# LGMOak/HighPerformanceComputing-LatticeBoltzmannMethod

Measured on NVIDIA B200. Metric: MLUPS (fp64 D2Q9), higher is better.
Workload: dtype f64

## Files before the change

highperformancecomputing-latticeboltzmannmethod_b200/csrc/lbm_tb.cu:

```cuda
#include <cstdlib>

#include "lbm_device.cuh"
#include "lbm_launch.cuh"
#include "lbm_tb.cuh"

namespace lbm {

namespace {

#ifndef TB_SKEW_THREADS
#define TB_SKEW_THREADS 512
#endif

template <int T, int B, bool FORCED, bool SKEW, bool FUSED>
__device__ __forceinline__ void tb_kernel_body(const TbArgs& a, int p2p) {
    extern __shared__ double ring[];
    pdl_wait();
    pdl_release();
    const bool edge_block = p2p && blockIdx.y < 2;
    if (edge_block) p2p_block_begin(a.px);
    tb_thread<T, B, FORCED, SKEW, FUSED>(a, ring, threadIdx.x, blockIdx.x, blockIdx.y);
    if (edge_block) p2p_block_end(a.px, gridDim.x * 2);
}

template <int T, int B, bool FORCED, bool SKEW = true, bool FUSED = false>
__global__ void __launch_bounds__(B, (T == 3 ? 384 : ((SKEW && T == 2) || T == 1 ? TB_SKEW_THREADS : 768)) / B)
    k_tb(const __grid_constant__ TbArgs a, int p2p) {
    tb_kernel_body<T, B, FORCED, SKEW, FUSED>(a, p2p);
}

__global__ void __launch_bounds__(256) k_macros_finish(ObserveArgs o, const double* __restrict__ m_rho,
                                                       const double* __restrict__ m_ux, const double* __restrict__ m_uy,
                                                       double* __restrict__ rho, double* __restrict__ ux,
                                                       double* __restrict__ uy) {
    __shared__ double t[3][32][33];
    const Layout& L = o.L;
    const int x0 = blockIdx.y * 32, y0 = blockIdx.x * 32;
    for (int k = threadIdx.y; k < 32; k += blockDim.y) {
        const int x = x0 + k, y = y0 + threadIdx.x;
        if (x < L.lnx && y < L.ny) {
            const long long g = (long long)x * L.ny + y;
            double r = m_rho[g], u = m_ux[g], v = m_uy[g];
            const bool on_in = o.bc.inlet && x == 0, on_out = o.bc.outlet && x == L.lnx - 1;
            if ((on_in || on_out) && !o.mask[L.at(x + 1, y)]) {
                double f[Q], rb = 0.0, uo = 0.0;
                current_from_next(o.cur, L, o.mask, o.bc, x, y, f, rb, uo);
                if (on_in) { r = rb; u = o.bc.u_in; v = 0.0; }
                if (on_out) { r = 1.0; u = uo; v = 0.0; }
            }
            t[0][k][threadIdx.x] = r;
            t[1][k][threadIdx.x] = u;
            t[2][k][threadIdx.x] = v;
        }
    }
    __syncthreads();
    for (int k = threadIdx.y; k < 32; k += blockDim.y) {
        const int x = x0 + threadIdx.x, y = y0 + k;
        if (x < L.lnx && y < L.ny) {
            const long long g = (long long)y * L.lnx + x;
            rho[g] = t[0][threadIdx.x][k];
            ux[g] = t[1][threadIdx.x][k];
            uy[g] = t[2][threadIdx.x][k];
        }
    }
}

inline int cdiv(long long a, long long b) { return (int)((a + b - 1) / b); }

int env_int(const char* name, int dflt) {
    const char* v = std::getenv(name);
    return v ? std::atoi(v) : dflt;
}

template <int T, int B, bool FORCED, bool SKEW = true, bool FUSED = false>
cudaError_t launch_one(TbArgs a, bool p2p, cudaStream_t s) {
    using S = TbShape<T, B>;
    auto kern = k_tb<T, B, FORCED, SKEW, FUSED>;
    const size_t smem = (size_t)S::RING_DOUBLES * sizeof(double) + (FUSED ? 16 : 0);
    static int slots = 0;
    if (!slots) {
        if (smem > 48 * 1024) {
            cudaError_t e = cudaFuncSetAttribute(kern, cudaFuncAttributeMaxDynamicSharedMemorySize, (int)smem);
            if (e != cudaSuccess) return e;
        }
        int per_sm = 0, dev = 0, sms = 0;
        cudaGetDevice(&dev);
        cudaDeviceGetAttribute(&sms, cudaDevAttrMultiProcessorCount, dev);
        cudaError_t e = cudaOccupancyMaxActiveBlocksPerMultiprocessor(&per_sm, kern, B, smem);
        if (e != cudaSuccess) return e;
        slots = (per_sm > 0 ? per_sm : 1) * (sms > 0 ? sms : 1);
    }
    const int lnx = a.L.lnx;
    const int strips = cdiv(a.L.ny, S::H);
    a.edge_cols = 0;
    a.x_begin = 0;
    a.x_end = lnx;
    if (p2p) {
        a.edge_cols = lnx / 2 < 8 ? lnx / 2 : 8;
        a.x_begin = a.edge_cols;
        a.x_end = lnx - a.edge_cols;
    }
    const int ncols = a.x_end - a.x_begin;
    int chunks = 0;
    if (ncols > 0) {
        int xc = env_int("LBM_B200_TB_XC", 0);
        if (xc <= 0) {
            xc = 64;
            while (xc > 16 && (long long)strips * cdiv(ncols, xc) < 2LL * slots) xc /= 2;
        }
        a.xc = xc;
        chunks = cdiv(ncols, xc);
    } else {
        a.xc = 1;
    }
    dim3 grid(strips, chunks + (p2p ? 2 : 0));
    if (grid.y == 0) return cudaSuccess;
    cudaLaunchConfig_t cfg = {};
    cfg.gridDim = grid;
    cfg.blockDim = dim3(B);
    cfg.dynamicSmemBytes = smem;
    cfg.stream = s;
    cudaLaunchAttribute attr[1];
    attr[0].id = cudaLaunchAttributeProgrammaticStreamSerialization;
    attr[0].val.programmaticStreamSerializationAllowed = 1;
    cfg.attrs = attr;
    cfg.numAttrs = pdl_enabled() ? 1 : 0;
    return cudaLaunchKernelEx(&cfg, kern, a, p2p ? 1 : 0);
}

template <int T, int B>
cudaError_t launch_forced(const TbArgs& a, bool p2p, cudaStream_t s) {
    const bool forced = (a.Fx != 0.0 || a.Fy != 0.0);
    static const bool skew = env_int("LBM_B200_TB_SKEW", 1) != 0;
    if (T == 2 && !forced && !skew) return launch_one<T, B, false, false>(a, p2p, s);
    static const bool fused = env_int("LBM_B200_TB_FUSED", 0) != 0;
    if (T == 3 && B == 128 && !forced && fused) return launch_one<T, B, false, true, true>(a, p2p, s);
    return forced ? launch_one<T, B, true>(a, p2p, s) : launch_one<T, B, false>(a, p2p, s);
}

int block_threads() {
    static const int b = [] {
        const int v = env_int("LBM_B200_TB_B", 128);
        return v == 256 ? 256 : (v == 64 ? 64 : 128);
    }();
    return b;
}

}

cudaError_t launch_tb(int depth, TbArgs a, bool p2p, cudaStream_t s) {
    const int b = block_threads();
    tb_fill_offsets(a);
    static const int pf = env_int("LBM_B200_TB_PF", 1), fast = env_int("LBM_B200_TB_FAST", 1);
    a.pf_dist = pf;
    a.fast_lane = fast;
    switch (depth) {
        case 1: return b == 128 ? launch_forced<1, 128>(a, p2p, s) : (b == 64 ? launch_forced<1, 64>(a, p2p, s) : launch_forced<1, 256>(a, p2p, s));
        case 2: return b == 128 ? launch_forced<2, 128>(a, p2p, s) : (b == 64 ? launch_forced<2, 64>(a, p2p, s) : launch_forced<2, 256>(a, p2p, s));
        case 3: return b == 128 ? launch_forced<3, 128>(a, p2p, s) : (b == 64 ? launch_forced<3, 64>(a, p2p, s) : launch_forced<3, 256>(a, p2p, s));
        default: return cudaErrorInvalidValue;
    }
}

bool tb_worthwhile(const Layout& L) {
    const int b = block_threads();
    const long long blocks = (long long)cdiv(L.ny, b - 4) * cdiv(L.lnx, 64);
    return blocks >= 2LL * 148 * (TB_SKEW_THREADS / b);
}

int tb_rows_per_block(int depth) {
    const int b = block_threads();
    return depth == 1 ? b : b - 4;
}

size_t tb_shared_bytes(int depth) {
    const int b = block_threads();
    return (size_t)(depth - 1) * TB_SLOTS * Q * b * sizeof(double);
}

cudaError_t launch_macros_finish(const ObserveArgs& o, const double* m_rho, const double* m_ux, const double* m_uy,
                                 double* rho, double* ux, double* uy, cudaStream_t s) {
    dim3 grid(cdiv(o.L.ny, 32), cdiv(o.L.lnx, 32));
    k_macros_finish<<<grid, dim3(32, 8), 0, s>>>(o, m_rho, m_ux, m_uy, rho, ux, uy);
    return cudaGetLastError();
}

}
```

highperformancecomputing-latticeboltzmannmethod_b200/csrc/lbm_tb.cuh:

```cuda
#pragma once

#include "lbm_cell.cuh"
#include "lbm_kernels.cuh"
#include "lbm_layout.h"

namespace lbm {

enum TbEdge {
    TB_EDGE_CONST = 0,
    TB_EDGE_HALO = 1,
    TB_EDGE_WRAP = 2
};

constexpr int TB_SLOTS = 4;
constexpr int TB_MAX_DEPTH = 3;

struct TbArgs {
    const double* src;
    double* dst;
    Layout L;
    double tau_inv, Fx, Fy;
    int* first_bad;
    int bad_iter;
    BcArgs bc;
    const unsigned char* mask;
    int mask_lo, mask_hi;
    int mask_ylo, mask_yhi;
    int west, east;
    int periodic_y;
    int pull;
    int write;
    int x_begin, x_end, xc;
    int edge_cols;
    int halo_w;
    double *m_rho, *m_ux, *m_uy;
    P2pArgs px;
    long long ld_off[Q], st_off[Q], col_bytes;
    long long pf_off[Q];
    int pf_dist;
    long long plane_mul[5];
    int fast_lane;
};

inline void tb_fill_offsets(TbArgs& a) {
    for (int i = 0; i < Q; ++i) {
        a.ld_off[i] = 8 * ((long long)i * a.L.plane - (long long)cxi(i) * a.L.PY - cyi(i));
        a.st_off[i] = 8 * (long long)i * a.L.plane;
        a.pf_off[i] = 8 * ((long long)i * a.L.plane - (long long)cxi(i) * a.L.PY);
    }
    a.col_bytes = 8 * (long long)a.L.PY;
    for (int k = 0; k < 5; ++k) a.plane_mul[k] = 8 * (long long)k * a.L.plane;
}

template <class P>
LBM_HD P tb_opaque(P p) {
#if defined(__CUDA_ARCH__)
    asm volatile("" : "+l"(p));
#endif
    return p;
}
LBM_HD int tb_opaque_int(int v) {
#if defined(__CUDA_ARCH__)
    v = __shfl_sync(0xffffffffu, v, threadIdx.x & 31);
#endif
    return v;
}

#if defined(__CUDA_ARCH__)
#define TB_SYNC() __syncthreads()
#define TB_LD(p, coherent) ((coherent) ? __ldcg(p) : __ldg(p))
#define TB_FLAG(ptr, v) atomicMin((ptr), (v))
#define TB_ST(ptr, v) asm volatile("st.global.f64 [%0], %1;" ::"l"(ptr), "d"(v) : "memory")
#define TB_COLD __device__ __host__ __noinline__
#define TB_PREFETCH_L2(p) asm volatile("prefetch.global.L2 [%0];" ::"l"(p))
#define TB_COUNT(which, n) ((void)0)
#else
void tb_host_sync();
void tb_host_flag(int* p, int v);
#define TB_SYNC() tb_host_sync()
#define TB_LD(p, coherent) (*(p))
#define TB_FLAG(ptr, v) tb_host_flag((ptr), (v))
#define TB_ST(ptr, v) (*reinterpret_cast<double*>(ptr) = (v))
#define TB_COLD inline
#define TB_PREFETCH_L2(p) ((void)(p))
void tb_host_count(int which, int n);
#define TB_COUNT(which, n) tb_host_count((which), (n))
#endif

LBM_HD int tb_wrap(int v, int n) {
    v %= n;
    return v < 0 ? v + n : v;
}

template <int T, int B>
struct TbShape {
    static constexpr int ROFF = (T == 1) ? 0 : 2;
    static constexpr int H = B - 2 * ROFF;
    static constexpr int RING_DOUBLES = (T - 1) * TB_SLOTS * Q * B;
    static_assert(T >= 1 && T <= TB_MAX_DEPTH, "depth");
    static_assert(ROFF >= T - 1, "row overlap");
};

LBM_HD void tb_chunk(const TbArgs& a, int chunk, int& x0, int& x1, bool& edge) {
    const int lnx = a.L.lnx;
    edge = false;
    if (a.edge_cols > 0) {
        if (chunk == 0) { x0 = 0; x1 = a.edge_cols; edge = true; return; }
        if (chunk == 1) { x0 = lnx - a.edge_cols; x1 = lnx; edge = true; return; }
        chunk -= 2;
    }
    x0 = a.x_begin + chunk * a.xc;
    x1 = x0 + a.xc < a.x_end ? x0 + a.xc : a.x_end;
}

struct TbCell {
    double f[Q];
    int kind;
    int m;
    int xr;
};

template <int T, int B>
struct TbRow {
    int tid, y, yr, row_kind;
    bool wall_b, wall_t, out_row, edge;
    bool strip_walls;
    int x0, x1;
    const char* srow;
    char* drow;
    bool on[T];
    const char* pf_seg;
    int pf_bytes;
    int pf_last;
};

template <int T>
LBM_HD int tb_col_kind(const TbArgs& a, int x0, int x1, int k, int c, int& xr) {
    const int grow = T - k;
    const int lnx = a.L.lnx;
    xr = c;
    if (c < x0 - grow || c >= x1 + grow) return 0;
    if (c >= 0 && c < lnx) return 1;
    const int mode = c < 0 ? a.west : a.east;
    if (mode == TB_EDGE_WRAP) { xr = tb_wrap(c, lnx); return 1; }
    if (mode == TB_EDGE_HALO) return 1;
    return (c == -1 || c == lnx) ? 2 : 0;
}

template <int T, int B, bool PLAIN>
LBM_HD void tb_classify(const TbArgs& a, const TbRow<T, B>& r, int k, int c, bool masked, TbCell& cell) {
    cell.kind = 0;
    cell.m = 0;
    cell.xr = c;
    if (!r.on[k - 1]) return;
    int col_kind = 1;
    if (!PLAIN) {
        col_kind = tb_col_kind<T>(a, r.x0, r.x1, k, c, cell.xr);
        if (col_kind == 0) return;
    }
    if (r.row_kind == 2) { cell.kind = 2; return; }
    if (!PLAIN && col_kind == 2) { cell.kind = 3; return; }
    cell.kind = 1;
    if (masked) {
        const int gx = cell.xr + 1;
        if (gx >= a.mask_lo && gx < a.mask_hi) {
            cell.m = a.mask[a.L.at(gx, r.yr)];
            if (cell.m == 2) cell.kind = 4;
        }
    }
}

template <int T, int B, bool PLAIN>
LBM_HD void tb_issue(const TbArgs& a, const TbRow<T, B>& r, int c, bool masked, TbCell& cell) {
    tb_classify<T, B, PLAIN>(a, r, 1, c, masked, cell);
    if (cell.kind != 1) return;
    const char* p = r.srow + (long long)(cell.xr + 1 + Layout::XO) * a.col_bytes;
    const bool coherent = PLAIN ? false : r.edge;
    if ((T > 1) || a.pull) {
#pragma unroll
        for (int i = 0; i < Q; ++i) cell.f[i] = TB_LD(reinterpret_cast<const double*>(p + a.ld_off[i]), coherent);
    } else {
#pragma unroll
        for (int i = 0; i < Q; ++i) cell.f[i] = TB_LD(reinterpret_cast<const double*>(p + a.st_off[i]), coherent);
    }
}

template <int T, int B, bool PLAIN>
LBM_HD void tb_from_ring(const TbArgs& a, const TbRow<T, B>& r, const double* ring, int k, int c, bool masked, TbCell& cell) {
    tb_classify<T, B, PLAIN>(a, r, k, c, masked, cell);
    if (cell.kind != 1) return;
    const double* g = ring + (k - 2) * (TB_SLOTS * Q * B) + r.tid;
    const double* gw = g + ((c - 1) & (TB_SLOTS - 1)) * (Q * B);
    const double* g0 = g + (c & (TB_SLOTS - 1)) * (Q * B);
    const double* ge = g + ((c + 1) & (TB_SLOTS - 1)) * (Q * B);
    cell.f[0] = g0[0 * B];
    cell.f[1] = gw[1 * B];
    cell.f[2] = g0[2 * B - 1];
    cell.f[3] = ge[3 * B];
    cell.f[4] = g0[4 * B + 1];
    cell.f[5] = gw[5 * B - 1];
    cell.f[6] = ge[6 * B - 1];
    cell.f[7] = ge[7 * B + 1];
    cell.f[8] = gw[8 * B + 1];
}

template <int B>
TB_COLD void tb_ring_const(double* w, const TbArgs& a, int which) {
    if (which == 3) {
#pragma unroll
        for (int i = 0; i < Q; ++i) w[i * B] = 0.0;
        return;
    }
    const double* v = which == 2 ? a.bc.e : a.bc.w;
#pragma unroll
    for (int i = 0; i < Q; ++i) w[i * B] = v[i];
}

template <int T, int B>
LBM_HD void tb_push(const TbArgs& a, const TbRow<T, B>& r, int c, const double* f) {
    const Layout& L = a.L;
    const int lnx = L.lnx;
    const int de = lnx - 1 - c, dw = c;
    if (a.px.peer_dst_east && de < a.halo_w) {
        double* q = a.px.peer_dst_east + L.at(-de, r.y);
        q[1 * L.plane] = f[1];
        q[5 * L.plane] = f[5];
        q[8 * L.plane] = f[8];
        if (de <= a.halo_w - 2) {
            q[0 * L.plane] = f[0];
            q[2 * L.plane] = f[2];
            q[4 * L.plane] = f[4];
        }
        if (de <= a.halo_w - 3) {
            q[3 * L.plane] = f[3];
            q[6 * L.plane] = f[6];
            q[7 * L.plane] = f[7];
        }
    }
    if (a.px.peer_dst_west && dw < a.halo_w) {
        double* q = a.px.peer_dst_west + L.at(lnx + 1 + dw, r.y);
        q[3 * L.plane] = f[3];
        q[6 * L.plane] = f[6];
        q[7 * L.plane] = f[7];
        if (dw <= a.halo_w - 2) {
            q[0 * L.plane] = f[0];
            q[2 * L.plane] = f[2];
            q[4 * L.plane] = f[4];
        }
        if (dw <= a.halo_w - 3) {
            q[1 * L.plane] = f[1];
            q[5 * L.plane] = f[5];
            q[8 * L.plane] = f[8];
        }
    }
}

template <int T, int B, bool FORCED, bool PLAIN>
LBM_HD bool tb_finish(const TbArgs& a, const TbRow<T, B>& r, double* ring, int k, int c, TbCell& cell) {
    const Layout& L = a.L;
    const int lnx = L.lnx, ny = L.ny;
    if (cell.kind == 0) return false;
    double* w = ring + (k - 1) * (TB_SLOTS * Q * B) + (c & (TB_SLOTS - 1)) * (Q * B) + r.tid;
    if (cell.kind != 1) {
        if (k < T) {
            tb_ring_const<B>(w, a, cell.kind);
        } else if (cell.kind == 4) {
            if (a.m_rho) {
                const long long g = (long long)c * ny + r.y;
                a.m_rho[g] = 1.0;
                a.m_ux[g] = 0.0;
                a.m_uy[g] = 0.0;
            }
            if (T == 1 && !a.pull && a.write) {
                char* q = r.drow + (long long)(c + 1 + Layout::XO) * a.col_bytes;
#pragma unroll
                for (int i = 0; i < Q; ++i) TB_ST(q + a.st_off[i], a.bc.w[i]);
            }
            if (!PLAIN && r.edge && a.write) tb_push<T, B>(a, r, c, a.bc.w);
        }
        return false;
    }
    bool bad = false;
    double* f = cell.f;
    const bool rules = (T > 1) || a.pull;
    if (rules && cell.m == 0) {
        if (r.strip_walls) {
            if (r.wall_b) wall_bottom(f);
            if (r.wall_t) wall_top(f);
        }
        if (!PLAIN) {
            if (a.bc.inlet && cell.xr == 0) (void)zou_he_inlet(f, a.bc.u_in);
            if (a.bc.outlet && cell.xr == lnx - 1) (void)zou_he_outlet(f);
        }
    }
    if (rules) {
#pragma unroll
        for (int i = 0; i < Q; ++i) bad |= unstable_value(f[i]);
    }
    if (cell.m != 0) {
        if (k < T) {
            tb_ring_const<B>(w, a, 4);
        } else {
            if (a.m_rho) {
                const long long g = (long long)c * ny + r.y;
                a.m_rho[g] = 1.0;
                a.m_ux[g] = 0.0;
                a.m_uy[g] = 0.0;
            }
            if (a.write) {
                char* q = r.drow + (long long)(c + 1 + Layout::XO) * a.col_bytes;
                if (T == 1 && !a.pull) {
#pragma unroll
                    for (int i = 0; i < Q; ++i) TB_ST(q + a.st_off[i], a.bc.w[i]);
                }
                if (!PLAIN && r.edge) tb_push<T, B>(a, r, c, a.bc.w);
            }
        }
        return bad;
    } else {
        const Moments mo = moments(f);
        if (k == T && a.m_rho) {
            const long long g = (long long)c * ny + r.y;
            a.m_rho[g] = mo.rho;
            a.m_ux[g] = mo.ux;
            a.m_uy[g] = mo.uy;
        }
        if (FORCED)
            bgk_forced(f, mo, a.tau_inv, a.Fx, a.Fy, f);
        else
            bgk(f, mo, a.tau_inv, f);
        if (k < T) {
#pragma unroll
            for (int i = 0; i < Q; ++i) w[i * B] = f[i];
            return bad;
        }
        if (!a.write) return bad;
        char* q = r.drow + (long long)(c + 1 + Layout::XO) * a.col_bytes;
#pragma unroll
        for (int i = 0; i < Q; ++i) TB_ST(q + a.st_off[i], f[i]);
    }
    if (!PLAIN && r.edge) tb_push<T, B>(a, r, c, f);
    return bad;
}

template <int T, int B>
LBM_HD void tb_prefetch_l2(const TbArgs& a, const char* seg, int bytes, int col) {
#if defined(__CUDA_ARCH__)
    if (col > a.L.lnx) return;
    const char* p = seg + (long long)(col + 1 + Layout::XO) * a.col_bytes;
#pragma unroll
    for (int i = 0; i < Q; ++i)
        asm volatile("cp.async.bulk.prefetch.L2.global [%0], %1;" ::"l"(p + a.pf_off[i]), "r"(bytes) : "memory");
#else
    (void)a; (void)seg; (void)bytes; (void)col;
#endif
}

template <int T, int B, bool FORCED, bool PLAIN>
LBM_HD void tb_step(const TbArgs& a, const TbRow<T, B>& r, double* ring, int s, bool issue_next, bool masked, TbCell& cur,
                    TbCell& nxt, bool bad[T]) {
    if (r.tid == 0 && r.pf_bytes > 0 && s + 1 + a.pf_dist <= r.pf_last) tb_prefetch_l2<T, B>(a, r.pf_seg, r.pf_bytes, s + 1 + a.pf_dist);
    if (issue_next) tb_issue<T, B, PLAIN>(a, r, s + 1, masked, nxt);
    bad[0] |= tb_finish<T, B, FORCED, PLAIN>(a, r, ring, 1, s, cur);
#pragma unroll
    for (int k = 2; k <= T; ++k) {
        TB_SYNC();
        tb_from_ring<T, B, PLAIN>(a, r, ring, k, s - (k - 1), masked, cur);
        bad[k - 1] |= tb_finish<T, B, FORCED, PLAIN>(a, r, ring, k, s - (k - 1), cur);
    }
}

template <int T, int B, bool FORCED, bool PLAIN>
LBM_HD void tb_step_skew(const TbArgs& a, const TbRow<T, B>& r, double* ring, int s, bool masked, bool bad[T]) {
    if (r.tid == 0 && r.pf_bytes > 0 && s + a.pf_dist <= r.pf_last) tb_prefetch_l2<T, B>(a, r.pf_seg, r.pf_bytes, s + a.pf_dist);
    TbCell first;
    tb_issue<T, B, PLAIN>(a, r, s, masked, first);
#pragma unroll
    for (int k = T; k >= 2; --k) {
        TbCell cell;
        tb_from_ring<T, B, PLAIN>(a, r, ring, k, s - 2 * (k - 1), masked, cell);
        bad[k - 1] |= tb_finish<T, B, FORCED, PLAIN>(a, r, ring, k, s - 2 * (k - 1), cell);
    }
    bad[0] |= tb_finish<T, B, FORCED, PLAIN>(a, r, ring, 1, s, first);
    if (T > 1) TB_SYNC();
}

LBM_HD void tb_chain_load(const char* pl, long long col_bytes, const long long* pm, double f[Q]) {
    const char* p0 = pl;
    const char* pw = tb_opaque(pl - col_bytes);
    const char* pe = tb_opaque(pl + col_bytes);
    f[0] = TB_LD(reinterpret_cast<const double*>(p0), false);
    pw = tb_opaque(pw + pm[1]);
    f[1] = TB_LD(reinterpret_cast<const double*>(pw), false);
    p0 = tb_opaque(p0 + pm[2]);
    f[2] = TB_LD(reinterpret_cast<const double*>(p0) - 1, false);
    pe = tb_opaque(pe + pm[3]);
    f[3] = TB_LD(reinterpret_cast<const double*>(pe), false);
    p0 = tb_opaque(p0 + pm[2]);
    f[4] = TB_LD(reinterpret_cast<const double*>(p0) + 1, false);
    pw = tb_opaque(pw + pm[4]);
    f[5] = TB_LD(reinterpret_cast<const double*>(pw) - 1, false);
    pe = tb_opaque(pe + pm[3]);
    f[6] = TB_LD(reinterpret_cast<const double*>(pe) - 1, false);
    pe = tb_opaque(pe + pm[1]);
    f[7] = TB_LD(reinterpret_cast<const double*>(pe) + 1, false);
    pw = tb_opaque(pw + pm[3]);
    f[8] = TB_LD(reinterpret_cast<const double*>(pw) + 1, false);
}
LBM_HD void tb_chain_store(char* ps, long long plane_bytes, const double f[Q]) {
    char* q = ps;
#pragma unroll
    for (int i = 0; i < Q; ++i) {
        TB_ST(q, f[i]);
        if (i + 1 < Q) q = tb_opaque(q + plane_bytes);
    }
}

template <bool FORCED>
LBM_HD bool tb_fast_cell(const TbArgs& a, bool strip_walls, bool wall_b, bool wall_t, double f[Q], Moments& mo) {
    if (strip_walls) {
        if (wall_b) wall_bottom(f);
        if (wall_t) wall_top(f);
    }
    bool u = false;
#pragma unroll
    for (int i = 0; i < Q; ++i) u |= unstable_value(f[i]);
    mo = moments(f);
    if (FORCED)
        bgk_forced(f, mo, a.tau_inv, a.Fx, a.Fy, f);
    else
        bgk(f, mo, a.tau_inv, f);
    return u;
}

template <int T, int B, bool FORCED>
LBM_HD void tb_fast_lane(const TbArgs& a, const TbRow<T, B>& r, double* ring, int s, const int s_end, bool bad[T]) {
    bool act[T];
#pragma unroll
    for (int k = 0; k < T; ++k) act[k] = r.on[k] && r.row_kind == 1;
    const long long plane_bytes = a.st_off[1];
    constexpr int PF_LINES = (B * 8 + 32 + 2 * 127) / 128;
    static_assert(Q * PF_LINES <= B || B < 128, "one prefetch line per thread (the emulation's small blocks: a hint only)");
    const char* pfp = nullptr;
    if (r.pf_bytes > 0 && r.tid < Q * PF_LINES) {
        const int pop = r.tid / PF_LINES, line = r.tid - pop * PF_LINES;
        const int skew = (int)(reinterpret_cast<unsigned long long>(r.pf_seg) & 127);
        if (line * 128 < r.pf_bytes + skew)
            pfp = tb_opaque(r.pf_seg - skew + a.pf_off[pop] + line * 128 + (long long)(s + a.pf_dist + 1 + Layout::XO) * a.col_bytes);
    }
    const char* pl = tb_opaque(r.srow + (long long)(s + 1 + Layout::XO) * a.col_bytes);
    char* ps = tb_opaque(r.drow + (long long)(s - 2 * (T - 1) + 1 + Layout::XO) * a.col_bytes);
    double* const rt = ring + r.tid;
    for (; s < s_end; ++s) {
        if (pfp && s + a.pf_dist <= r.pf_last) TB_PREFETCH_L2(pfp);
        bool now[T];
#pragma unroll
        for (int k = 1; k <= T; ++k) {
            const int c = s - 2 * (k - 1);
            now[k - 1] = act[k - 1] && c >= r.x0 - (T - k) && c < r.x1 + (T - k);
        }
        double f1[Q];
        if (now[0]) tb_chain_load(pl, a.col_bytes, a.plane_mul, f1);
#pragma unroll
        for (int k = T; k >= 2; --k) {
            if (!now[k - 1]) continue;
            const int c = s - 2 * (k - 1);
            const double* g = rt + (k - 2) * (TB_SLOTS * Q * B);
            const double* gw = g + ((c - 1) & (TB_SLOTS - 1)) * (Q * B);
            const double* g0 = g + (c & (TB_SLOTS - 1)) * (Q * B);
            const double* ge = g + ((c + 1) & (TB_SLOTS - 1)) * (Q * B);
            double f[Q];
            f[0] = g0[0 * B];
            f[1] = gw[1 * B];
            f[2] = g0[2 * B - 1];
            f[3] = ge[3 * B];
            f[4] = g0[4 * B + 1];
            f[5] = gw[5 * B - 1];
            f[6] = ge[6 * B - 1];
            f[7] = ge[7 * B + 1];
            f[8] = gw[8 * B + 1];
            Moments mo;
            bad[k - 1] |= tb_fast_cell<FORCED>(a, r.strip_walls, r.wall_b, r.wall_t, f, mo);
            if (k < T) {
                double* w = rt + (k - 1) * (TB_SLOTS * Q * B) + (c & (TB_SLOTS - 1)) * (Q * B);
#pragma unroll
                for (int i = 0; i < Q; ++i) w[i * B] = f[i];
            } else {
                if (a.m_rho) {
                    const long long g = (long long)c * a.L.ny + r.y;
                    a.m_rho[g] = mo.rho;
                    a.m_ux[g] = mo.ux;
                    a.m_uy[g] = mo.uy;
                }
                tb_chain_store(ps, plane_bytes, f);
            }
        }
        if (now[0]) {
            Moments mo;
            bad[0] |= tb_fast_cell<FORCED>(a, r.strip_walls, r.wall_b, r.wall_t, f1, mo);
            if (T > 1) {
                double* w = rt + (s & (TB_SLOTS - 1)) * (Q * B);
#pragma unroll
                for (int i = 0; i < Q; ++i) w[i * B] = f1[i];
            } else {
                if (a.m_rho) {
                    const long long g = (long long)s * a.L.ny + r.y;
                    a.m_rho[g] = mo.rho;
                    a.m_ux[g] = mo.ux;
                    a.m_uy[g] = mo.uy;
                }
                tb_chain_store(ps, plane_bytes, f1);
            }
        }
        pl = tb_opaque(pl + a.col_bytes);
        ps = tb_opaque(ps + a.col_bytes);
        if (pfp) pfp = tb_opaque(pfp + a.col_bytes);
        if (T > 1) TB_SYNC();
    }
}

template <int T, int B, bool FORCED>
LBM_HD void tb_fast_lane_fused(const TbArgs& a, const TbRow<T, B>& r, double* ring, int s, const int s_end, bool bad[T]) {
    constexpr int K = T > 1 ? T - 1 : 1;
    bool act[T];
#pragma unroll
    for (int k = 0; k < T; ++k) act[k] = r.on[k] && r.row_kind == 1;
    const long long plane_bytes = a.st_off[1];
    constexpr int PF_LINES = (B * 8 + 32 + 2 * 127) / 128;
    const char* pfp = nullptr;
    if (r.pf_bytes > 0 && r.tid < Q * PF_LINES) {
        const int pop = r.tid / PF_LINES, line = r.tid - pop * PF_LINES;
        const int skew = (int)(reinterpret_cast<unsigned long long>(r.pf_seg) & 127);
        if (line * 128 < r.pf_bytes + skew)
            pfp = tb_opaque(r.pf_seg - skew + a.pf_off[pop] + line * 128 + (long long)(s + a.pf_dist + 1 + Layout::XO) * a.col_bytes);
    }
    const char* pl = tb_opaque(r.srow + (long long)(s + 1 + Layout::XO) * a.col_bytes);
    char* ps = tb_opaque(r.drow + (long long)(s - 2 * (T - 1) + 1 + Layout::XO) * a.col_bytes);
    double* const rt = ring + r.tid;
    for (; s < s_end; ++s) {
        if (pfp && s + a.pf_dist <= r.pf_last) TB_PREFETCH_L2(pfp);
        double f1[Q];
        if (act[0]) tb_chain_load(pl, a.col_bytes, a.plane_mul, f1);
        double f[K][Q], rho[K], mx[K], my[K];
        Moments mo[K];
        bool window = true;
#pragma unroll
        for (int j = K - 1; j >= 0; --j) {
            const int c = s - 2 * (j + 1);
            const double* g = rt + j * (TB_SLOTS * Q * B);
            const double* gw = g + ((c - 1) & (TB_SLOTS - 1)) * (Q * B);
            const double* g0 = g + (c & (TB_SLOTS - 1)) * (Q * B);
            const double* ge = g + ((c + 1) & (TB_SLOTS - 1)) * (Q * B);
            f[j][0] = g0[0 * B];
            f[j][1] = gw[1 * B];
            f[j][2] = g0[2 * B - 1];
            f[j][3] = ge[3 * B];
            f[j][4] = g0[4 * B + 1];
            f[j][5] = gw[5 * B - 1];
            f[j][6] = ge[6 * B - 1];
            f[j][7] = ge[7 * B + 1];
            f[j][8] = gw[8 * B + 1];
        }
        if (r.strip_walls) {
#pragma unroll
            for (int j = 0; j < K; ++j) {
                if (r.wall_b) wall_bottom(f[j]);
                if (r.wall_t) wall_top(f[j]);
            }
        }
#pragma unroll
        for (int j = K - 1; j >= 0; --j) {
            bool u = false;
#pragma unroll
            for (int i = 0; i < Q; ++i) u |= unstable_value(f[j][i]);
            bad[j + 1] |= u && act[j + 1];
            moment_sums(f[j], rho[j], mx[j], my[j]);
            window = window && div_pair_window(mx[j], my[j], rho[j]);
        }
        if (window) {
#pragma unroll
            for (int j = K - 1; j >= 0; --j) {
                mo[j].rho = rho[j];
                div_pair_core(mx[j], my[j], rho[j], mo[j].ux, mo[j].uy);
            }
        } else {
#pragma unroll
            for (int j = K - 1; j >= 0; --j) {
                mo[j].rho = rho[j];
                div_pair(mx[j], my[j], rho[j], mo[j].ux, mo[j].uy);
            }
        }
#pragma unroll
        for (int j = K - 1; j >= 0; --j) {
            if (FORCED)
                bgk_forced(f[j], mo[j], a.tau_inv, a.Fx, a.Fy, f[j]);
            else
                bgk(f[j], mo[j], a.tau_inv, f[j]);
        }
#pragma unroll
        for (int j = K - 1; j >= 0; --j) {
            if (!act[j + 1]) continue;
            const int c = s - 2 * (j + 1);
            if (j + 2 < T) {
                double* w = rt + (j + 1) * (TB_SLOTS * Q * B) + (c & (TB_SLOTS - 1)) * (Q * B);
#pragma unroll
                for (int i = 0; i < Q; ++i) w[i * B] = f[j][i];
            } else {
                if (a.m_rho) {
                    const long long g = (long long)c * a.L.ny + r.y;
                    a.m_rho[g] = mo[j].rho;
                    a.m_ux[g] = mo[j].ux;
                    a.m_uy[g] = mo[j].uy;
                }
                tb_chain_store(ps, plane_bytes, f[j]);
            }
        }
        if (act[0]) {
            Moments m1;
            bad[0] |= tb_fast_cell<FORCED>(a, r.strip_walls, r.wall_b, r.wall_t, f1, m1);
            double* w = rt + (s & (TB_SLOTS - 1)) * (Q * B);
#pragma unroll
            for (int i = 0; i < Q; ++i) w[i * B] = f1[i];
        }
        pl = tb_opaque(pl + a.col_bytes);
        ps = tb_opaque(ps + a.col_bytes);
        if (pfp) pfp = tb_opaque(pfp + a.col_bytes);
        TB_SYNC();
    }
}

template <int T, int B, bool FORCED, bool SKEW = true, bool FUSED = false>
LBM_HD void tb_thread(const TbArgs& a, double* ring, int tid_, int strip_, int chunk_) {
    using S = TbShape<T, B>;
    const int tid = tb_opaque_int(tid_), strip = tb_opaque_int(strip_), chunk = tb_opaque_int(chunk_);
    const int ny = a.L.ny, lnx = a.L.lnx;
    TbRow<T, B> r;
    tb_chunk(a, chunk, r.x0, r.x1, r.edge);
    if (r.x0 >= r.x1) return;

    r.tid = tid;
    r.y = strip * S::H - S::ROFF + tid;
    r.yr = r.y;
    if (a.periodic_y) {
        r.row_kind = (r.y >= -(T - 1) && r.y < ny + (T - 1)) ? 1 : 0;
        r.yr = tb_wrap(r.y, ny);
    } else {
        r.row_kind = (r.y >= 0 && r.y < ny) ? 1 : ((r.y == -1 || r.y == ny) ? 2 : 0);
    }
    r.wall_b = a.bc.walls && r.yr == 0;
    r.wall_t = a.bc.walls && r.yr == ny - 1;
    {
        const int lo = strip * S::H - S::ROFF, hi = lo + B;
        r.strip_walls = a.bc.walls && ((lo <= 0 && hi > 0) || (lo <= ny - 1 && hi > ny - 1) || a.periodic_y);
    }
    r.out_row = (tid >= S::ROFF && tid < S::ROFF + S::H && r.y >= 0 && r.y < ny);
#pragma unroll
    for (int k = 1; k <= T; ++k) {
        const int grow = T - k;
        r.on[k - 1] = r.row_kind != 0 && tid >= S::ROFF - grow && tid < S::ROFF + S::H + grow && (k < T || r.out_row);
    }
    r.srow = tb_opaque(reinterpret_cast<const char*>(a.src + (Layout::YO + r.yr)));
    r.drow = tb_opaque(reinterpret_cast<char*>(a.dst + (Layout::YO + r.y)));
    r.pf_bytes = 0;
    r.pf_seg = nullptr;
    if (a.pf_dist > 0) {
        int first = strip * S::H - S::ROFF - 1;
        int last = first + B + 2;
        if (first < -Layout::YO) first = -Layout::YO;
        if (last > a.L.PY - Layout::YO) last = a.L.PY - Layout::YO;
        first &= ~1;
        last = (last + 1) & ~1;
        if (last > first) {
            r.pf_seg = reinterpret_cast<const char*>(a.src + (Layout::YO + first));
            r.pf_bytes = (last - first) * 8;
        }
    }
    bool bad[T];
#pragma unroll
    for (int k = 0; k < T; ++k) bad[k] = false;

    const int c_lo = (a.west == TB_EDGE_CONST && a.bc.inlet) ? 1 : 0;
    const int c_hi = (a.east == TB_EDGE_CONST && a.bc.outlet) ? lnx - 1 : lnx;
    if (SKEW) {
        const int s_first = r.x0 - (T - 1), s_last = r.x1 - 1 + 2 * (T - 1);
        int p0 = (r.x0 > c_lo ? r.x0 : c_lo) + 2 * (T - 1);
        int p1 = (r.x1 + (T - 2) < c_hi - 1 ? r.x1 + (T - 2) : c_hi - 1) + 1;
        if (r.edge) p1 = p0;
        r.pf_last = r.x1 + (T - 2) < lnx ? r.x1 + (T - 2) : lnx;
        int m0 = a.mask_lo - 1, m1 = a.mask_hi - 1 + 2 * (T - 1);
        {
            const int lo = strip * S::H - S::ROFF;
            if (!a.periodic_y && (lo >= a.mask_yhi || lo + B <= a.mask_ylo)) m1 = m0;
        }
        if (T > 1 && r.row_kind == 2) {
#pragma unroll
            for (int k = 1; k < T; ++k) {
                if (!r.on[k - 1]) continue;
                for (int slot = 0; slot < TB_SLOTS; ++slot)
                    tb_ring_const<B>(ring + (k - 1) * (TB_SLOTS * Q * B) + slot * (Q * B) + r.tid, a, 2);
            }
        }
        const bool fast = a.write && ((T > 1) || a.pull) && a.fast_lane;
        int q0 = p0, q1 = p1;
        if (!r.edge && r.x0 - (T - 1) >= c_lo && r.x1 + (T - 1) <= c_hi) { q0 = s_first; q1 = s_last + 1; }
        if (!fast) q1 = q0;
        int s = s_first;
        while (s <= s_last) {
            if (s >= q0 && s < q1 && !(s >= m0 && s < m1)) {
                const int e = (s < m0 && m0 < q1) ? m0 : q1;
                if (tid == 0) TB_COUNT(0, e - s);
                if constexpr (FUSED && T > 2) {
                    const int f0 = s > p0 ? s : p0, f1 = e < p1 ? e : p1;
                    const bool any = f0 < f1;
#pragma unroll 1
                    for (int seg = 0; seg < 3; ++seg) {
                        const int to = !any ? e : (seg == 0 ? f0 : (seg == 1 ? f1 : e));
                        if (s >= to) continue;
                        if (seg == 1 && any) tb_fast_lane_fused<T, B, FORCED>(a, r, ring, s, to, bad);
                        else tb_fast_lane<T, B, FORCED>(a, r, ring, s, to, bad);
                        s = to;
                    }
                } else {
                    tb_fast_lane<T, B, FORCED>(a, r, ring, s, e, bad);
                }
                s = e;
                continue;
            }
            if (tid == 0) TB_COUNT(1, 1);
            tb_step_skew<T, B, FORCED, false>(a, r, ring, s, true, bad);
            ++s;
        }
    } else {
    const int s_first = r.x0 - (T - 1), s_last = r.x1 + (T - 2);
    int p0 = r.x0 + (T - 1), p1 = s_last;
    if (p0 < c_lo + (T - 1)) p0 = c_lo + (T - 1);
    if (p1 > c_hi - 1) p1 = c_hi - 1;
    if (r.edge) p1 = p0;
    r.pf_last = s_last < lnx ? s_last : lnx;
    TbCell ca, cb;
    tb_issue<T, B, false>(a, r, s_first, true, ca);
    int s = s_first;
    bool a_is_cur = true;
    const int m0 = a.mask_lo - 2, m1 = a.mask_hi - 1 + (T - 1);
    while (s <= s_last) {
        if (a_is_cur && s >= p0 && s + 1 < p1) {
            for (; s + 1 < p1; s += 2) {
                tb_step<T, B, FORCED, true>(a, r, ring, s, true, s >= m0 && s < m1, ca, cb, bad);
                tb_step<T, B, FORCED, true>(a, r, ring, s + 1, true, s + 1 >= m0 && s + 1 < m1, cb, ca, bad);
            }
            continue;
        }
        if (a_is_cur) tb_step<T, B, FORCED, false>(a, r, ring, s, s < s_last, true, ca, cb, bad);
        else tb_step<T, B, FORCED, false>(a, r, ring, s, s < s_last, true, cb, ca, bad);
        a_is_cur = !a_is_cur;
        ++s;
    }
    }
#pragma unroll
    for (int k = 0; k < T; ++k)
        if (bad[k]) TB_FLAG(a.first_bad, a.bad_iter + k);
}

cudaError_t launch_tb(int depth, TbArgs a, bool p2p, cudaStream_t s);
cudaError_t launch_macros_finish(const ObserveArgs& o, const double* m_rho, const double* m_ux, const double* m_uy,
                                 double* rho, double* ux, double* uy, cudaStream_t s);
bool tb_worthwhile(const Layout& L);
int tb_rows_per_block(int depth);
size_t tb_shared_bytes(int depth);

}
```

Measured before the change: 87100.

## Restructure temporal-blocking shared ring into per-direction-group slots to shrink shared memory

Replaces the 4-slot × 9-population shared-memory ring per temporal level with a layout grouped by x-direction (east/zero/west populations), each group holding only the slots it needs (2, 3, 4). That cuts shared-memory use from 36 to 27 planes per level. Slot offsets are precomputed once and advanced incrementally each column instead of being recomputed with masks. The launch bounds for non-fused depth-3 kernels are raised to request more resident threads per SM, trading possible register pressure or spills for occupancy.

```diff
diff --git a/highperformancecomputing-latticeboltzmannmethod_b200/csrc/lbm_tb.cu b/highperformancecomputing-latticeboltzmannmethod_b200/csrc/lbm_tb.cu
--- a/highperformancecomputing-latticeboltzmannmethod_b200/csrc/lbm_tb.cu
+++ b/highperformancecomputing-latticeboltzmannmethod_b200/csrc/lbm_tb.cu
@@ -24,7 +24,7 @@
 }
 
 template <int T, int B, bool FORCED, bool SKEW = true, bool FUSED = false>
-__global__ void __launch_bounds__(B, (T == 3 ? 384 : ((SKEW && T == 2) || T == 1 ? TB_SKEW_THREADS : 768)) / B)
+__global__ void __launch_bounds__(B, (T == 3 ? (FUSED ? 384 : TB_SKEW_THREADS) : ((SKEW && T == 2) || T == 1 ? TB_SKEW_THREADS : 768)) / B)
     k_tb(const __grid_constant__ TbArgs a, int p2p) {
     tb_kernel_body<T, B, FORCED, SKEW, FUSED>(a, p2p);
 }
@@ -76,7 +76,7 @@
 cudaError_t launch_one(TbArgs a, bool p2p, cudaStream_t s) {
     using S = TbShape<T, B>;
     auto kern = k_tb<T, B, FORCED, SKEW, FUSED>;
-    const size_t smem = (size_t)S::RING_DOUBLES * sizeof(double) + (FUSED ? 16 : 0);
+    const size_t smem = (size_t)S::RING_DOUBLES * sizeof(double);
     static int slots = 0;
     if (!slots) {
         if (smem > 48 * 1024) {
@@ -175,7 +175,7 @@
 
 size_t tb_shared_bytes(int depth) {
     const int b = block_threads();
-    return (size_t)(depth - 1) * TB_SLOTS * Q * b * sizeof(double);
+    return (size_t)(depth - 1) * TB_RING_PLANES * b * sizeof(double);
 }
 
 cudaError_t launch_macros_finish(const ObserveArgs& o, const double* m_rho, const double* m_ux, const double* m_uy,
diff --git a/highperformancecomputing-latticeboltzmannmethod_b200/csrc/lbm_tb.cuh b/highperformancecomputing-latticeboltzmannmethod_b200/csrc/lbm_tb.cuh
--- a/highperformancecomputing-latticeboltzmannmethod_b200/csrc/lbm_tb.cuh
+++ b/highperformancecomputing-latticeboltzmannmethod_b200/csrc/lbm_tb.cuh
@@ -12,8 +12,61 @@
     TB_EDGE_WRAP = 2
 };
 
-constexpr int TB_SLOTS = 4;
 constexpr int TB_MAX_DEPTH = 3;
+
+constexpr int TB_RING_PLANES = 27;
+
+LBM_HD constexpr int tb_ring_slots(int g) { return g + 2; }
+
+template <int B>
+LBM_HD constexpr int tb_ring_at(int k, int g, int s) {
+    const int n = tb_ring_slots(g);
+    int slot = s % n;
+    if (slot < 0) slot += n;
+    return ((k - 1) * TB_RING_PLANES + 3 * (g * (g + 3) / 2 + slot)) * B;
+}
+
+template <int B>
+LBM_HD int tb_ring_slot(int g, int s) {
+    return tb_ring_at<B>(1, g, s) - tb_ring_at<B>(1, g, 0);
+}
+
+template <int B>
+LBM_HD void tb_ring_pull(const double* rt, int k, int o0, int o1, int o2, double f[Q]) {
+    const double* e = rt + tb_ring_at<B>(k, 0, 0) + o0;
+    const double* z = rt + tb_ring_at<B>(k, 1, 0) + o1;
+    const double* w = rt + tb_ring_at<B>(k, 2, 0) + o2;
+    f[7] = e[1];
+    f[3] = e[B];
+    f[6] = e[2 * B - 1];
+    f[4] = z[1];
+    f[0] = z[B];
+    f[2] = z[2 * B - 1];
+    f[8] = w[1];
+    f[1] = w[B];
+    f[5] = w[2 * B - 1];
+}
+template <int B>
+LBM_HD void tb_ring_put(double* rt, int k, int o0, int o1, int o2, const double f[Q]) {
+    double* e = rt + tb_ring_at<B>(k, 0, 0) + o0;
+    double* z = rt + tb_ring_at<B>(k, 1, 0) + o1;
+    double* w = rt + tb_ring_at<B>(k, 2, 0) + o2;
+    e[0] = f[7];
+    e[B] = f[3];
+    e[2 * B] = f[6];
+    z[0] = f[4];
+    z[B] = f[0];
+    z[2 * B] = f[2];
+    w[0] = f[8];
+    w[B] = f[1];
+    w[2 * B] = f[5];
+}
+
+template <int B>
+LBM_HD void tb_ring_fill(double* rt, int k, const double f[Q]) {
+#pragma unroll 1
+    for (int s = 0; s < tb_ring_slots(2); ++s) tb_ring_put<B>(rt, k, tb_ring_slot<B>(0, s), tb_ring_slot<B>(1, s), tb_ring_slot<B>(2, s), f);
+}
 
 struct TbArgs {
     const double* src;
@@ -96,7 +149,7 @@
 struct TbShape {
     static constexpr int ROFF = (T == 1) ? 0 : 2;
     static constexpr int H = B - 2 * ROFF;
-    static constexpr int RING_DOUBLES = (T - 1) * TB_SLOTS * Q * B;
+    static constexpr int RING_DOUBLES = tb_ring_at<B>(T, 0, 0);
     static_assert(T >= 1 && T <= TB_MAX_DEPTH, "depth");
     static_assert(ROFF >= T - 1, "row overlap");
 };
@@ -185,35 +238,42 @@
     }
 }
 
+struct TbSlots {
+    int st[3], pl[3];
+};
+template <int B>
+LBM_HD TbSlots tb_slots(int s, bool skew) {
+    TbSlots o;
+#pragma unroll
+    for (int g = 0; g < 3; ++g) {
+        o.st[g] = tb_ring_slot<B>(g, s);
+        o.pl[g] = tb_ring_slot<B>(g, s + (skew ? 1 : 2));
+    }
+    return o;
+}
+template <int B>
+LBM_HD void tb_slots_advance(TbSlots& o) {
+#pragma unroll
+    for (int g = 0; g < 3; ++g) {
+        o.st[g] = o.pl[g];
+        o.pl[g] = o.pl[g] + 3 * B == tb_ring_slots(g) * 3 * B ? 0 : o.pl[g] + 3 * B;
+    }
+}
+
 template <int T, int B, bool PLAIN>
-LBM_HD void tb_from_ring(const TbArgs& a, const TbRow<T, B>& r, const double* ring, int k, int c, bool masked, TbCell& cell) {
+LBM_HD void tb_from_ring(const TbArgs& a, const TbRow<T, B>& r, const double* ring, int k, int c, const TbSlots& o,
+                         bool masked, TbCell& cell) {
     tb_classify<T, B, PLAIN>(a, r, k, c, masked, cell);
     if (cell.kind != 1) return;
-    const double* g = ring + (k - 2) * (TB_SLOTS * Q * B) + r.tid;
-    const double* gw = g + ((c - 1) & (TB_SLOTS - 1)) * (Q * B);
-    const double* g0 = g + (c & (TB_SLOTS - 1)) * (Q * B);
-    const double* ge = g + ((c + 1) & (TB_SLOTS - 1)) * (Q * B);
-    cell.f[0] = g0[0 * B];
-    cell.f[1] = gw[1 * B];
-    cell.f[2] = g0[2 * B - 1];
-    cell.f[3] = ge[3 * B];
-    cell.f[4] = g0[4 * B + 1];
-    cell.f[5] = gw[5 * B - 1];
-    cell.f[6] = ge[6 * B - 1];
-    cell.f[7] = ge[7 * B + 1];
-    cell.f[8] = gw[8 * B + 1];
+    tb_ring_pull<B>(ring + r.tid, k - 1, o.pl[0], o.pl[1], o.pl[2], cell.f);
 }
 
 template <int B>
-TB_COLD void tb_ring_const(double* w, const TbArgs& a, int which) {
-    if (which == 3) {
-#pragma unroll
-        for (int i = 0; i < Q; ++i) w[i * B] = 0.0;
-        return;
-    }
-    const double* v = which == 2 ? a.bc.e : a.bc.w;
-#pragma unroll
-    for (int i = 0; i < Q; ++i) w[i * B] = v[i];
+TB_COLD void tb_ring_const(double* rt, int k, int o0, int o1, int o2, const TbArgs& a, int which) {
+    double v[Q];
+#pragma unroll
+    for (int i = 0; i < Q; ++i) v[i] = which == 3 ? 0.0 : (which == 2 ? a.bc.e[i] : a.bc.w[i]);
+    tb_ring_put<B>(rt, k, o0, o1, o2, v);
 }
 
 template <int T, int B>
@@ -256,14 +316,13 @@
 }
 
 template <int T, int B, bool FORCED, bool PLAIN>
-LBM_HD bool tb_finish(const TbArgs& a, const TbRow<T, B>& r, double* ring, int k, int c, TbCell& cell) {
+LBM_HD bool tb_finish(const TbArgs& a, const TbRow<T, B>& r, double* ring, int k, int c, const TbSlots& o, TbCell& cell) {
     const Layout& L = a.L;
     const int lnx = L.lnx, ny = L.ny;
     if (cell.kind == 0) return false;
-    double* w = ring + (k - 1) * (TB_SLOTS * Q * B) + (c & (TB_SLOTS - 1)) * (Q * B) + r.tid;
     if (cell.kind != 1) {
         if (k < T) {
-            tb_ring_const<B>(w, a, cell.kind);
+            tb_ring_const<B>(ring + r.tid, k, o.st[0], o.st[1], o.st[2], a, cell.kind);
         } else if (cell.kind == 4) {
             if (a.m_rho) {
                 const long long g = (long long)c * ny + r.y;
@@ -299,7 +358,7 @@
     }
     if (cell.m != 0) {
         if (k < T) {
-            tb_ring_const<B>(w, a, 4);
+            tb_ring_const<B>(ring + r.tid, k, o.st[0], o.st[1], o.st[2], a, 4);
         } else {
             if (a.m_rho) {
                 const long long g = (long long)c * ny + r.y;
@@ -330,8 +389,7 @@
         else
             bgk(f, mo, a.tau_inv, f);
         if (k < T) {
-#pragma unroll
-            for (int i = 0; i < Q; ++i) w[i * B] = f[i];
+            tb_ring_put<B>(ring + r.tid, k, o.st[0], o.st[1], o.st[2], f);
             return bad;
         }
         if (!a.write) return bad;
@@ -361,12 +419,13 @@
                     TbCell& nxt, bool bad[T]) {
     if (r.tid == 0 && r.pf_bytes > 0 && s + 1 + a.pf_dist <= r.pf_last) tb_prefetch_l2<T, B>(a, r.pf_seg, r.pf_bytes, s + 1 + a.pf_dist);
     if (issue_next) tb_issue<T, B, PLAIN>(a, r, s + 1, masked, nxt);
-    bad[0] |= tb_finish<T, B, FORCED, PLAIN>(a, r, ring, 1, s, cur);
+    const TbSlots o = tb_slots<B>(s, false);
+    bad[0] |= tb_finish<T, B, FORCED, PLAIN>(a, r, ring, 1, s, o, cur);
 #pragma unroll
     for (int k = 2; k <= T; ++k) {
         TB_SYNC();
-        tb_from_ring<T, B, PLAIN>(a, r, ring, k, s - (k - 1), masked, cur);
-        bad[k - 1] |= tb_finish<T, B, FORCED, PLAIN>(a, r, ring, k, s - (k - 1), cur);
+        tb_from_ring<T, B, PLAIN>(a, r, ring, k, s - (k - 1), o, masked, cur);
+        bad[k - 1] |= tb_finish<T, B, FORCED, PLAIN>(a, r, ring, k, s - (k - 1), o, cur);
     }
 }
 
@@ -375,13 +434,14 @@
     if (r.tid == 0 && r.pf_bytes > 0 && s + a.pf_dist <= r.pf_last) tb_prefetch_l2<T, B>(a, r.pf_seg, r.pf_bytes, s + a.pf_dist);
     TbCell first;
     tb_issue<T, B, PLAIN>(a, r, s, masked, first);
+    const TbSlots o = tb_slots<B>(s, true);
 #pragma unroll
     for (int k = T; k >= 2; --k) {
         TbCell cell;
-        tb_from_ring<T, B, PLAIN>(a, r, ring, k, s - 2 * (k - 1), masked, cell);
-        bad[k - 1] |= tb_finish<T, B, FORCED, PLAIN>(a, r, ring, k, s - 2 * (k - 1), cell);
-    }
-    bad[0] |= tb_finish<T, B, FORCED, PLAIN>(a, r, ring, 1, s, first);
+        tb_from_ring<T, B, PLAIN>(a, r, ring, k, s - 2 * (k - 1), o, masked, cell);
+        bad[k - 1] |= tb_finish<T, B, FORCED, PLAIN>(a, r, ring, k, s - 2 * (k - 1), o, cell);
+    }
+    bad[0] |= tb_finish<T, B, FORCED, PLAIN>(a, r, ring, 1, s, o, first);
     if (T > 1) TB_SYNC();
 }
 
@@ -451,6 +511,7 @@
     const char* pl = tb_opaque(r.srow + (long long)(s + 1 + Layout::XO) * a.col_bytes);
     char* ps = tb_opaque(r.drow + (long long)(s - 2 * (T - 1) + 1 + Layout::XO) * a.col_bytes);
     double* const rt = ring + r.tid;
+    TbSlots o = tb_slots<B>(s, true);
     for (; s < s_end; ++s) {
         if (pfp && s + a.pf_dist <= r.pf_last) TB_PREFETCH_L2(pfp);
         bool now[T];
@@ -465,26 +526,12 @@
         for (int k = T; k >= 2; --k) {
             if (!now[k - 1]) continue;
             const int c = s - 2 * (k - 1);
-            const double* g = rt + (k - 2) * (TB_SLOTS * Q * B);
-            const double* gw = g + ((c - 1) & (TB_SLOTS - 1)) * (Q * B);
-            const double* g0 = g + (c & (TB_SLOTS - 1)) * (Q * B);
-            const double* ge = g + ((c + 1) & (TB_SLOTS - 1)) * (Q * B);
             double f[Q];
-            f[0] = g0[0 * B];
-            f[1] = gw[1 * B];
-            f[2] = g0[2 * B - 1];
-            f[3] = ge[3 * B];
-            f[4] = g0[4 * B + 1];
-            f[5] = gw[5 * B - 1];
-            f[6] = ge[6 * B - 1];
-            f[7] = ge[7 * B + 1];
-            f[8] = gw[8 * B + 1];
+            tb_ring_pull<B>(rt, k - 1, o.pl[0], o.pl[1], o.pl[2], f);
             Moments mo;
             bad[k - 1] |= tb_fast_cell<FORCED>(a, r.strip_walls, r.wall_b, r.wall_t, f, mo);
             if (k < T) {
-                double* w = rt + (k - 1) * (TB_SLOTS * Q * B) + (c & (TB_SLOTS - 1)) * (Q * B);
-#pragma unroll
-                for (int i = 0; i < Q; ++i) w[i * B] = f[i];
+                tb_ring_put<B>(rt, k, o.st[0], o.st[1], o.st[2], f);
             } else {
                 if (a.m_rho) {
                     const long long g = (long long)c * a.L.ny + r.y;
@@ -499,9 +546,7 @@
             Moments mo;
             bad[0] |= tb_fast_cell<FORCED>(a, r.strip_walls, r.wall_b, r.wall_t, f1, mo);
             if (T > 1) {
-                double* w = rt + (s & (TB_SLOTS - 1)) * (Q * B);
-#pragma unroll
-                for (int i = 0; i < Q; ++i) w[i * B] = f1[i];
+                tb_ring_put<B>(rt, 1, o.st[0], o.st[1], o.st[2], f1);
             } else {
                 if (a.m_rho) {
                     const long long g = (long long)s * a.L.ny + r.y;
@@ -515,6 +560,7 @@
         pl = tb_opaque(pl + a.col_bytes);
         ps = tb_opaque(ps + a.col_bytes);
         if (pfp) pfp = tb_opaque(pfp + a.col_bytes);
+        tb_slots_advance<B>(o);
         if (T > 1) TB_SYNC();
     }
 }
@@ -537,6 +583,7 @@
     const char* pl = tb_opaque(r.srow + (long long)(s + 1 + Layout::XO) * a.col_bytes);
     char* ps = tb_opaque(r.drow + (long long)(s - 2 * (T - 1) + 1 + Layout::XO) * a.col_bytes);
     double* const rt = ring + r.tid;
+    TbSlots o = tb_slots<B>(s, true);
     for (; s < s_end; ++s) {
         if (pfp && s + a.pf_dist <= r.pf_last) TB_PREFETCH_L2(pfp);
         double f1[Q];
@@ -545,22 +592,7 @@
         Moments mo[K];
         bool window = true;
 #pragma unroll
-        for (int j = K - 1; j >= 0; --j) {
-            const int c = s - 2 * (j + 1);
-            const double* g = rt + j * (TB_SLOTS * Q * B);
-            const double* gw = g + ((c - 1) & (TB_SLOTS - 1)) * (Q * B);
-            const double* g0 = g + (c & (TB_SLOTS - 1)) * (Q * B);
-            const double* ge = g + ((c + 1) & (TB_SLOTS - 1)) * (Q * B);
-            f[j][0] = g0[0 * B];
-            f[j][1] = gw[1 * B];
-            f[j][2] = g0[2 * B - 1];
-            f[j][3] = ge[3 * B];
-            f[j][4] = g0[4 * B + 1];
-            f[j][5] = gw[5 * B - 1];
-            f[j][6] = ge[6 * B - 1];
-            f[j][7] = ge[7 * B + 1];
-            f[j][8] = gw[8 * B + 1];
-        }
+        for (int j = K - 1; j >= 0; --j) tb_ring_pull<B>(rt, j + 1, o.pl[0], o.pl[1], o.pl[2], f[j]);
         if (r.strip_walls) {
 #pragma unroll
             for (int j = 0; j < K; ++j) {
@@ -602,9 +634,7 @@
             if (!act[j + 1]) continue;
             const int c = s - 2 * (j + 1);
             if (j + 2 < T) {
-                double* w = rt + (j + 1) * (TB_SLOTS * Q * B) + (c & (TB_SLOTS - 1)) * (Q * B);
-#pragma unroll
-                for (int i = 0; i < Q; ++i) w[i * B] = f[j][i];
+                tb_ring_put<B>(rt, j + 2, o.st[0], o.st[1], o.st[2], f[j]);
             } else {
                 if (a.m_rho) {
                     const long long g = (long long)c * a.L.ny + r.y;
@@ -618,13 +648,12 @@
         if (act[0]) {
             Moments m1;
             bad[0] |= tb_fast_cell<FORCED>(a, r.strip_walls, r.wall_b, r.wall_t, f1, m1);
-            double* w = rt + (s & (TB_SLOTS - 1)) * (Q * B);
-#pragma unroll
-            for (int i = 0; i < Q; ++i) w[i * B] = f1[i];
+            tb_ring_put<B>(rt, 1, o.st[0], o.st[1], o.st[2], f1);
         }
         pl = tb_opaque(pl + a.col_bytes);
         ps = tb_opaque(ps + a.col_bytes);
         if (pfp) pfp = tb_opaque(pfp + a.col_bytes);
+        tb_slots_advance<B>(o);
         TB_SYNC();
     }
 }
@@ -694,11 +723,8 @@
         }
         if (T > 1 && r.row_kind == 2) {
 #pragma unroll
-            for (int k = 1; k < T; ++k) {
-                if (!r.on[k - 1]) continue;
-                for (int slot = 0; slot < TB_SLOTS; ++slot)
-                    tb_ring_const<B>(ring + (k - 1) * (TB_SLOTS * Q * B) + slot * (Q * B) + r.tid, a, 2);
-            }
+            for (int k = 1; k < T; ++k)
+                if (r.on[k - 1]) tb_ring_fill<B>(ring + r.tid, k, a.bc.e);
         }
         const bool fast = a.write && ((T > 1) || a.pull) && a.fast_lane;
         int q0 = p0, q1 = p1;
```

Result: faster. 90300, median of 6 (+3.7%).
